# hormes/koordinator

Measured on AMD Instinct MI355X. Metric: pod×node Filter+Score evals/sec + pods/sec at 50k nodes, 1/2/4/8 GPUs, higher is better.
Workload: dtype int64

## Files before the change

koordinator_amd/csrc/gs_kernels.hip:

```cpp
#include <hip/hip_runtime.h>
#include <stdint.h>

#include <cstdio>
#include <vector>

#include "gs_eval_dev.h"

namespace gs {

__device__ __forceinline__ uint32_t node_prep_flags(uint32_t sf, int64_t update_time, int64_t now, int32_t filter_expired,
                                                    int32_t has_exp, int64_t exp_ns) {
  bool exists = sf & SF_METRIC;
  bool expired = !exists || !(sf & SF_UPDATE_TIME) || (exp_ns > 0 && now - update_time >= exp_ns);
  bool skip_filter = !exists || (filter_expired && has_exp && expired);
  uint32_t df = 0;
  if (!skip_filter) {
    const uint32_t npd = ((sf & SF_NP_MEM) ? 1u : 0u) | ((sf & SF_NP_AGG) ? 2u : 0u);
    if (sf & SF_FAIL_NP) df |= DF_LA_FAIL_NP | npd << DF_NP_DETAIL_SHIFT;
    if (sf & SF_PROD_THR) {
      if (sf & SF_FAIL_P) df |= DF_LA_FAIL_P | (((sf & SF_P_MEM) ? 1u : 0u) << DF_P_DETAIL_SHIFT);
    } else if (sf & SF_FAIL_NP) {
      df |= DF_LA_FAIL_P | npd << DF_P_DETAIL_SHIFT;
    }
  }
// ... 263 lines not shown
      if (nz && lane < ls) {
        s_score[nb] = b;
        s_count[nb] = (int32_t)c;
        slot_of[b] = (int8_t)nb;
      }
      if (sm) {
        next = __builtin_amdgcn_readlane(b, ls);
        nlev += __popcll(nzm & ((1ull << ls) - 1ull));
        break;
      }
      nlev += __popcll(nzm);
      cum += (uint32_t)wave_sum((int)c);
    }
    for (int j = nlev + lane; j < LEVALL; j += 64) { s_score[j] = -1; s_count[j] = 0; }
    if (lane == 0) {
      s_nlev = nlev;
      s_next = next;
    }
  } else if (t == 64 && cp.tb) {
    tiebreak_records(cp.seed, cp.seq[k], cp.tb + (size_t)k * TB_N);
  }
  __syncthreads();
  CT(2);
  const int nlev = s_nlev;
  for (int e = t; e < W * LEVALL; e += CAND_THREADS) {
    const int w = e / LEVALL, j = e % LEVALL;
    uint32_t off = 0;
    if (j < nlev) {
      for (int jj = 0; jj < j; ++jj) off += s_count[jj];
      for (int ww = 0; ww < w; ++ww) off += whist[ww * nbins + s_score[j]];
    }
    s_woff[w][j] = off;
  }
  __syncthreads();
  CT(3);
  uint32_t* out = lists + (size_t)k * lcap;
  if (nlev > 0) {
    uint32_t run_l = lane < LEVALL ? s_woff[wave][lane] : 0;
    const int thr = s_score[nlev - 1];
    auto next_step = [&](uint32_t b) {
      for (; b < we; b += 512) {
        const uint32_t st = (b - wb) / 512;
        if (st >= (uint32_t)STEPCAP || s_stepmax[wave][st] >= thr) break;
      }
      return b;
    };
    constexpr int PD = 4;
    uint32_t bq[PD];
    int4 vq[PD];
    uint32_t nb = next_step(wb);
#pragma unroll
    for (int u = 0; u < PD; ++u) {
      bq[u] = nb;
      vq[u] = nb < we ? row4[(nb + lane * 8) / 8] : make_int4(-1, -1, -1, -1);
      nb = nb < we ? next_step(nb + 512) : we;
    }
    while (bq[0] < we) {
      const uint32_t base = bq[0];
      const int4 q = vq[0];
#pragma unroll
      for (int u = 0; u + 1 < PD; ++u) { bq[u] = bq[u + 1]; vq[u] = vq[u + 1]; }
      bq[PD - 1] = nb;
      vq[PD - 1] = nb < we ? row4[(nb + lane * 8) / 8] : make_int4(-1, -1, -1, -1);
      nb = nb < we ? next_step(nb + 512) : we;
      const int16_t* e = reinterpret_cast<const int16_t*>(&q);
      int slot[8];
      uint32_t present = 0;
#pragma unroll
      for (int x = 0; x < 8; ++x) {
        slot[x] = e[x] >= thr ? slot_of[e[x]] : -1;
        if (slot[x] >= 0) present |= 1u << slot[x];
      }
      uint32_t pw = (uint32_t)wave_or((int)present);
      for (; pw; pw &= pw - 1) {
        const int j = __ffs(pw) - 1;
        int c = 0;
#pragma unroll
        for (int x = 0; x < 8; ++x) c += slot[x] == j;
        const int incl = wave_incl_scan(c);
        int pos = __builtin_amdgcn_readlane((int)run_l, j) + incl - c;
#pragma unroll
        for (int x = 0; x < 8; ++x)
          if (slot[x] == j) out[pos++] = n0 + base + lane * 8 + x;
        const int tot = __builtin_amdgcn_readlane(incl, 63);
        if (lane == j) run_l += tot;
      }
    }
  }
  CT(4);
  if (t == 0) {
    LevelHdr h;
    h.nlev = nlev < MAXLEV ? nlev : MAXLEV;
    h.feasible = (int32_t)s_total;
    h.next = nlev > MAXLEV ? s_score[MAXLEV] : s_next;
    int32_t tot = 0;
    for (int j = 0; j < MAXLEV; ++j) { h.score[j] = s_score[j]; h.count[j] = s_count[j]; tot += s_count[j]; }
    h.total = tot;
    hdrs[k] = h;
    LevelExt x;
    x.nlev = nlev;
    x.next = s_next;
    for (int j = 0; j < LEVX; ++j) { x.score[j] = s_score[MAXLEV + j]; x.count[j] = s_count[MAXLEV + j]; }
    ext[k] = x;
  }
}

__global__ void __launch_bounds__(256) cs_hist_kernel(const int16_t* __restrict__ S, uint32_t ld, uint32_t lenv,
                                                      int nbins, uint32_t slice, int G, uint32_t* __restrict__ ghist) {
  extern __shared__ __align__(16) uint32_t hist[];
  const int g = blockIdx.x, k = blockIdx.y, t = threadIdx.x;
  for (int b = t; b < nbins; b += 256) hist[b] = 0;
  __syncthreads();
  const uint32_t b0 = (uint32_t)g * slice, b1 = min(lenv, b0 + slice);
  const int4* row4 = reinterpret_cast<const int4*>(S + (size_t)k * ld);
  for (uint32_t i = b0 + t * 8; i < b1; i += 2 * 2048) {
    const int4 q0 = row4[i / 8];
    const int4 q1 = i + 2048 < b1 ? row4[(i + 2048) / 8] : make_int4(-1, -1, -1, -1);
    const int16_t* e0 = reinterpret_cast<const int16_t*>(&q0);
    const int16_t* e1 = reinterpret_cast<const int16_t*>(&q1);
#pragma unroll
    for (int x = 0; x < 8; ++x) {
      if (e0[x] >= 0) atomicAdd(&hist[e0[x]], 1u);
      if (e1[x] >= 0) atomicAdd(&hist[e1[x]], 1u);
    }
  }
  __syncthreads();
  uint32_t* out = ghist + ((size_t)k * G + g) * nbins;
  for (int b = t; b < nbins; b += 256) out[b] = hist[b];
}

__global__ void __launch_bounds__(256) cs_pick_kernel(const uint32_t* __restrict__ ghist, int nbins, int G, int lcap,
                                                      uint32_t* __restrict__ offs, LevelHdr* __restrict__ hdrs,
                                                      LevelExt* __restrict__ ext) {
  extern __shared__ __align__(16) uint32_t comb[];
  __shared__ uint32_t s_total;
  __shared__ int32_t s_nlev, s_next, s_score[LEVALL], s_count[LEVALL];
  __shared__ uint32_t s_v[CS_GMAX][LEVALL];
  const int k = blockIdx.x, t = threadIdx.x, wave = t >> 6, lane = t & 63;
  const uint32_t* h = ghist + (size_t)k * G * nbins;
  for (int b = t; b < nbins; b += 256) comb[b] = 0;
  if (t == 0) s_total = 0;
  __syncthreads();
  const int tot = G * nbins;
  for (int e0 = t; e0 < tot; e0 += 4 * 256) {
    uint32_t v[4];
#pragma unroll
    for (int u = 0; u < 4; ++u) v[u] = e0 + u * 256 < tot ? h[e0 + u * 256] : 0u;
#pragma unroll
    for (int u = 0; u < 4; ++u)
      if (v[u]) atomicAdd(&comb[(e0 + u * 256) % nbins], v[u]);
  }
  __syncthreads();
  {
    uint32_t s = 0;
    for (int b = t; b < nbins; b += 256) s += comb[b];
    s = (uint32_t)wave_sum((int)s);
    if (lane == 0 && s) atomicAdd(&s_total, s);
  }
  if (wave == 0) {
    const uint32_t target = (uint32_t)k + 1;
    const uint64_t lt = (1ull << lane) - 1ull;
    int nlev = 0, next = -1;
    uint32_t cum = 0;
    for (int hi = nbins - 1; hi >= 0; hi -= 64) {
      const int b = hi - lane;
      const uint32_t c = b >= 0 ? comb[b] : 0u;
      const bool nz = c != 0;
      const uint64_t nzm = __ballot(nz);
      if (!nzm) continue;
      const uint32_t cb = cum + (uint32_t)(wave_incl_scan((int)c) - (int)c);
      const int nb = nlev + __popcll(nzm & lt);
      const bool stop = nz && (nb == LEVALL || cb + c > (uint32_t)lcap || cb >= target);
      const uint64_t sm = __ballot(stop);
      const int ls = sm ? __builtin_ctzll(sm) : 64;
      if (nz && lane < ls) {
        s_score[nb] = b;
        s_count[nb] = (int32_t)c;
      }
      if (sm) {
        next = __builtin_amdgcn_readlane(b, ls);
        nlev += __popcll(nzm & ((1ull << ls) - 1ull));
        break;
      }
      nlev += __popcll(nzm);
      cum += (uint32_t)wave_sum((int)c);
    }
    for (int j = nlev + lane; j < LEVALL; j += 64) { s_score[j] = -1; s_count[j] = 0; }
    if (lane == 0) {
      s_nlev = nlev;
      s_next = next;
    }
  }
  __syncthreads();
  const int nlev = s_nlev;
  for (int e = t; e < G * LEVALL; e += 256) {
    const int g = e / LEVALL, j = e % LEVALL;
    s_v[g][j] = j < nlev ? h[(size_t)g * nbins + s_score[j]] : 0u;
  }
  __syncthreads();
  if (t < LEVALL) {
    uint32_t base = 0;
    for (int jj = 0; jj < t && jj < nlev; ++jj) base += (uint32_t)s_count[jj];
    uint32_t* o = offs + (size_t)k * G * LEVALL;
    for (int g = 0; g < G; ++g) {
      o[g * LEVALL + t] = base;
      base += s_v[g][t];
    }
  }
  if (t == 0) {
    LevelHdr hd;
    hd.nlev = nlev < MAXLEV ? nlev : MAXLEV;
    hd.feasible = (int32_t)s_total;
    hd.next = nlev > MAXLEV ? s_score[MAXLEV] : s_next;
    int32_t sum = 0;
    for (int j = 0; j < MAXLEV; ++j) { hd.score[j] = s_score[j]; hd.count[j] = s_count[j]; sum += s_count[j]; }
    hd.total = sum;
    hdrs[k] = hd;
    LevelExt x;
    x.nlev = nlev;
    x.next = s_next;
    for (int j = 0; j < LEVX; ++j) { x.score[j] = s_score[MAXLEV + j]; x.count[j] = s_count[MAXLEV + j]; }
    ext[k] = x;
  }
}

__global__ void __launch_bounds__(64) cs_list_kernel(const int16_t* __restrict__ S, uint32_t ld, uint32_t lenv,
                                                     uint32_t n0, int nbins, uint32_t slice, int G, int lcap,
                                                     const uint32_t* __restrict__ offs,
                                                     const LevelHdr* __restrict__ hdrs,
                                                     const LevelExt* __restrict__ ext, uint32_t* __restrict__ lists) {
  extern __shared__ __align__(16) int8_t slot_of[];
  const int g = blockIdx.x, k = blockIdx.y, lane = threadIdx.x;
  const int nlev = ext[k].nlev;
  if (nlev <= 0) return;
  for (int b = lane; b < nbins; b += 64) slot_of[b] = -1;
  __syncthreads();
  int sc = -1;
  if (lane < nlev) sc = lane < MAXLEV ? hdrs[k].score[lane] : ext[k].score[lane - MAXLEV];
  if (lane < nlev) slot_of[sc] = (int8_t)lane;
  const int thr = __shfl(sc, nlev - 1);
  __syncthreads();
  uint32_t run_l = lane < LEVALL ? offs[((size_t)k * G + g) * LEVALL + lane] : 0u;
  uint32_t* out = lists + (size_t)k * lcap;
  const uint32_t b0 = (uint32_t)g * slice, b1 = min(lenv, b0 + slice);
  const int4* row4 = reinterpret_cast<const int4*>(S + (size_t)k * ld);
  for (uint32_t gb = b0; gb < b1; gb += 4 * 512) {
    int4 qs[4];
#pragma unroll
    for (int u = 0; u < 4; ++u)
      qs[u] = gb + u * 512 < b1 ? row4[(gb + u * 512 + lane * 8) / 8] : make_int4(-1, -1, -1, -1);
#pragma unroll
    for (int u = 0; u < 4; ++u) {
      const uint32_t base = gb + u * 512;
      const int16_t* e = reinterpret_cast<const int16_t*>(&qs[u]);
      int slot[8];
      uint32_t present = 0;
#pragma unroll
      for (int x = 0; x < 8; ++x) {
        slot[x] = e[x] >= thr ? slot_of[e[x]] : -1;
        if (slot[x] >= 0) present |= 1u << slot[x];
      }
      uint32_t pw = (uint32_t)wave_or((int)present);
      for (; pw; pw &= pw - 1) {
        const int j = __ffs(pw) - 1;
        int c = 0;
#pragma unroll
        for (int x = 0; x < 8; ++x) c += slot[x] == j;
        const int incl = wave_incl_scan(c);
        int pos = __builtin_amdgcn_readlane((int)run_l, j) + incl - c;
#pragma unroll
        for (int x = 0; x < 8; ++x)
          if (slot[x] == j) out[pos++] = n0 + base + lane * 8 + x;
        const int tot = __builtin_amdgcn_readlane(incl, 63);
        if (lane == j) run_l += tot;
      }
    }
  }
}

constexpr int FIX_THREADS = 256;
__device__ __forceinline__ int lower_bound_u32(const uint32_t* a, int n, uint32_t x) {
  int lo = 0;
  while (n > 0) {
    const int h = n >> 1;
    if (a[lo + h] < x) { lo += h + 1; n -= h + 1; } else { n = h; }
  }
  return lo;
}
__global__ void __launch_bounds__(FIX_THREADS) fix_levels_kernel(int16_t* __restrict__ S, uint32_t ld, int max_score,
                                                                 int lcap, uint32_t* __restrict__ lists,
                                                                 LevelHdr* __restrict__ hdrs, LevelExt* __restrict__ ext,
                                                                 CandPatch cp, uint64_t* stamps) {
  uint64_t ct_last = stamps ? __builtin_amdgcn_s_memtime() : 0;
  auto CT = [&](int i) {
    if (!stamps) return;
    const uint64_t t_ = __builtin_amdgcn_s_memtime();
    if (threadIdx.x == 0) atomicAdd(reinterpret_cast<unsigned long long*>(&stamps[i]), (unsigned long long)(t_ - ct_last));
    ct_last = t_;
  };
  extern __shared__ __align__(16) uint32_t smem[];
  const int nbins = max_score + 1;
  uint32_t* hist = smem;
  uint32_t* olist = smem + nbins;
  __shared__ uint32_t p_raw[MAX_BATCH], p_node[MAX_BATCH];
  __shared__ int32_t p_old[MAX_BATCH], p_new[MAX_BATCH];
  __shared__ unsigned long long m_old[LEVALL][2], m_new[LEVALL][2];
  __shared__ int32_t n_ol[LEVALL];
  __shared__ int32_t o_score[LEVALL], o_count[LEVALL], o_off[LEVALL];
  __shared__ int32_t n_score[LEVALL], n_count[LEVALL], n_off[LEVALL];
  __shared__ int32_t s_onlev, s_onext, s_ofeas, s_np, s_fd, s_nlev, s_next, s_top;
  __shared__ int32_t r_old[MAX_BATCH], r_new[MAX_BATCH], p_sidx[MAX_BATCH];
  __shared__ int32_t s_wd[2];
  int8_t* lev_of = reinterpret_cast<int8_t*>(olist + lcap);
  const int k = blockIdx.x, t = threadIdx.x, lane = t & 63;
  if (cp.prev_committed[0] <= 0) return;
  const int32_t* lh = reinterpret_cast<const int32_t*>(cp.landed);
  const int nl = min(max(lh[0], 0), MAX_BATCH), npol = min(max(lh[1], 0), nl);
  const int split = min(max(npol, nl - 64), 64);
  const int slot_t = t < 64 ? (t < split ? t : -1) : (t < 128 && split + (t - 64) < nl ? split + (t - 64) : -1);
  const int32_t node_t = slot_t >= 0 ? lh[LANDED_NODES / 4 + slot_t] : -1;
  __shared__ unsigned int s_ev_max[2];
  if (stamps && t < 2) s_ev_max[t] = 0;
  if (stamps) __syncthreads();
  static_assert(FIX_THREADS == 256 && MAX_BATCH <= 128, "fix_levels_kernel: waves 0-1 evaluate, 2-3 load");
  if (t >= FIX_THREADS - 64) {
    const LevelHdr& h = hdrs[k];
    const LevelExt& x = ext[k];
    const int onl = x.nlev;
    const int j = lane;
    int sc = -1, cnt = 0;
    if (j < LEVALL) {
      sc = j < MAXLEV ? h.score[j] : x.score[j - MAXLEV];
      cnt = j < onl ? (j < MAXLEV ? h.count[j] : x.count[j - MAXLEV]) : 0;
    }
    const int incl = wave_incl_scan(cnt);
    if (j < LEVALL) {
      o_score[j] = sc;
      o_count[j] = cnt;
      o_off[j] = incl - cnt;
    }
    if (lane == 0) {
      s_onlev = onl;
      s_onext = x.next;
      s_ofeas = h.feasible;
      s_fd = 0;
      s_top = onl > 0 ? h.score[0] : x.next;
    }
    const int otot = onl > 0 ? __shfl(incl, onl - 1) : 0;
    const uint32_t* src = lists + (size_t)k * lcap;
    for (int e0 = 0; e0 < otot; e0 += 8 * 64) {
      uint32_t v[8];
#pragma unroll
      for (int u = 0; u < 8; ++u) {
        const int e = e0 + u * 64 + lane;
        v[u] = e < otot ? src[e] : 0u;
      }
#pragma unroll
      for (int u = 0; u < 8; ++u) {
        const int e = e0 + u * 64 + lane;
        if (e < otot) olist[e] = v[u];
      }
    }
  } else if (t >= FIX_THREADS - 128) {
    for (int b = lane; b < nbins; b += 64) hist[b] = cp.hist[(size_t)k * nbins + b];
  }
  const bool numa = (cp.pf.enabled & 0x30u) != 0;
  size_t at = 0;
  int so = -1, sn = -1, aff_v = -1;
  bool valid = false;
  if (t < 128) {
    const int32_t node = node_t;
    valid = node >= 0 && (uint32_t)node >= cp.n0 && (uint32_t)node < cp.n1;
    p_raw[t] = valid ? (uint32_t)node : 0xffffffffu;
    if (valid) {
      const uint64_t e0 = stamps ? __builtin_amdgcn_s_memtime() : 0;
      if (stamps && t == 0)
        atomicAdd(reinterpret_cast<unsigned long long*>(&stamps[10]), (unsigned long long)(e0 - ct_last));
      at = (size_t)k * ld + ((uint32_t)node - cp.n0);
      so = S[at];
      const Row r = reinterpret_cast<const Row*>(cp.landed + LANDED_ROWS)[slot_t];
      if (stamps) {
        __builtin_amdgcn_s_waitcnt(0);
        atomicMax(&s_ev_max[0], (unsigned int)(__builtin_amdgcn_s_memtime() - e0));
      }
      const PairOut o = eval_pair<false, true, true>(r, cp.pods[k], cp.pf, cp.m);
      sn = total_score(o, cp.pf);
      if (numa && ((r.nr.nflags >> NF_POLICY_SHIFT) & 3u)) aff_v = o.code ? 0 : (int)o.aff;
      if (stamps) atomicMax(&s_ev_max[1], (unsigned int)(__builtin_amdgcn_s_memtime() - e0));
    }
    r_old[t] = so;
    r_new[t] = sn;
  }
  __syncthreads();
  if (stamps && t == 0) {
    atomicAdd(reinterpret_cast<unsigned long long*>(&stamps[8]), (unsigned long long)s_ev_max[0]);
    atomicAdd(reinterpret_cast<unsigned long long*>(&stamps[9]), (unsigned long long)s_ev_max[1]);
    atomicAdd(reinterpret_cast<unsigned long long*>(&stamps[11]),
              (unsigned long long)(__builtin_amdgcn_s_memtime() - ct_last));
  }
  if (t < 128) {
    const uint32_t x = p_raw[t];
    const uint32_t k0 = p_raw[lane], k1 = p_raw[64 + lane];
    int rank = 0;
#pragma unroll
    for (int i = 0; i < 64; ++i) {
      const uint32_t y0 = __builtin_amdgcn_readlane(k0, i), y1 = __builtin_amdgcn_readlane(k1, i);
      rank += ((y0 < x || (y0 == x && i < t))) ? 1 : 0;
      rank += ((y1 < x || (y1 == x && 64 + i < t))) ? 1 : 0;
    }
    p_sidx[rank] = t;
  }
  __syncthreads();
  bool keep = false;
  int idx = 0, wpre = 0;
  uint32_t xs = 0;
  if (t < 2 * 64) {
    idx = p_sidx[t];
    xs = p_raw[idx];
    keep = xs != 0xffffffffu && (t == 0 || p_raw[p_sidx[t - 1]] != xs);
    const uint64_t m = __ballot(keep);
    wpre = __popcll(m & ((1ull << lane) - 1ull));
    if (lane == 0) s_wd[t >> 6] = __popcll(m);
  }
  __syncthreads();
  if (keep) {
    const int pos = (t >= 64 ? s_wd[0] : 0) + wpre;
    const int o_ = r_old[idx], n_ = r_new[idx];
    p_node[pos] = xs;
    p_old[pos] = o_;
    p_new[pos] = n_;
    if (o_ >= 0) atomicSub(&hist[o_], 1u);
    if (n_ >= 0) atomicAdd(&hist[n_], 1u);
    const int fd = (n_ >= 0 ? 1 : 0) - (o_ >= 0 ? 1 : 0);
    if (fd) atomicAdd(&s_fd, fd);
    atomicMax(&s_top, n_);
  }
  if (t == 0) s_np = s_wd[0] + s_wd[1];
  __syncthreads();
  CT(5);
  const int np = s_np;
  if (t < 64) {
    const uint32_t target = (uint32_t)k + 1;
    const int onext = s_onext;
    const uint64_t lt = (1ull << lane) - 1ull;
    int nlev = 0, next = -1;
    uint32_t cum = 0;
    for (int hi = min(s_top, nbins - 1); hi >= 0; hi -= 64) {
      const int b = hi - lane;
      const uint32_t c = b >= 0 ? hist[b] : 0u;
      const bool nz = c != 0;
      const uint64_t nzm = __ballot(nz);
      if (!nzm) continue;
      const uint32_t cb = cum + (uint32_t)(wave_incl_scan((int)c) - (int)c);
      const int nb = nlev + __popcll(nzm & lt);
      const bool stop = nz && (nb == LEVALL || cb + c > (uint32_t)lcap || cb >= target || b <= onext);
      const uint64_t sm = __ballot(stop);
      const int ls = sm ? __builtin_ctzll(sm) : 64;
      if (nz && lane < ls) {
        n_score[nb] = b;
        n_count[nb] = (int32_t)c;
      }
      if (sm) {
        next = __builtin_amdgcn_readlane(b, ls);
        nlev += __popcll(nzm & ((1ull << ls) - 1ull));
        break;
      }
      nlev += __popcll(nzm);
      cum += (uint32_t)wave_sum((int)c);
    }
    for (int j = nlev + lane; j < LEVALL; j += 64) { n_score[j] = -1; n_count[j] = 0; }
    WAVE_FENCE();
    const int cnt = lane < LEVALL ? n_count[lane] : 0;
    if (lane < LEVALL) n_off[lane] = wave_incl_scan(cnt) - cnt;
    if (lane == 0) {
      s_nlev = nlev;
      s_next = next;
    }
  }
  __syncthreads();
  CT(6);
  const int nlev = s_nlev;
  for (int b = t; b < nbins; b += FIX_THREADS) lev_of[b] = -1;
  if (t < LEVALL * 2) { m_old[t >> 1][t & 1] = 0; m_new[t >> 1][t & 1] = 0; }
  __syncthreads();
  if (t < nlev) {
    lev_of[n_score[t]] = (int8_t)t;
    int o = -1;
    for (int i = 0; i < s_onlev; ++i) o = o_score[i] == n_score[t] ? i : o;
    n_ol[t] = o;
  }
  __syncthreads();
  if (t < np) {
    const int jo = p_old[t] >= 0 ? lev_of[p_old[t]] : -1, jn = p_new[t] >= 0 ? lev_of[p_new[t]] : -1;
    if (jo >= 0) atomicOr(&m_old[jo][t >> 6], 1ull << (t & 63));
    if (jn >= 0) atomicOr(&m_new[jn][t >> 6], 1ull << (t & 63));
  }
  __syncthreads();
  auto below = [](const unsigned long long (&m)[2], int pos) {
    const int lo = min(pos, 64), hi = max(pos - 64, 0);
    return __popcll(lo >= 64 ? m[0] : (m[0] & ((1ull << lo) - 1ull))) +
           __popcll(hi >= 64 ? m[1] : (m[1] & ((1ull << hi) - 1ull)));
  };
  uint32_t* out = lists + (size_t)k * lcap;
  const int onlev = s_onlev;
  const int otot = onlev > 0 ? o_off[onlev - 1] + o_count[onlev - 1] : 0;
  for (int e = t; e < otot; e += FIX_THREADS) {
    int oj = 0;
    for (int step = 16; step; step >>= 1)
      if (oj + step < onlev && o_off[oj + step] <= e) oj += step;
    const int j = lev_of[o_score[oj]];
    if (j < 0) continue;
    const uint32_t x = olist[e];
    const int pos = lower_bound_u32(p_node, np, x);
    if (pos < np && p_node[pos] == x) continue;
    out[n_off[j] + (e - o_off[oj]) - below(m_old[j], pos) + below(m_new[j], pos)] = x;
  }
  if (t < np) {
    const int sn = p_new[t];
    const int j = sn >= 0 ? lev_of[sn] : -1;
    if (j >= 0) {
      const int oj = n_ol[j];
      const int before = oj >= 0 ? lower_bound_u32(olist + o_off[oj], o_count[oj], p_node[t]) - below(m_old[j], t) : 0;
      out[n_off[j] + below(m_new[j], t) + before] = p_node[t];
    }
  }
  CT(7);
  if (t == 0) {
    LevelHdr h;
    h.nlev = nlev < MAXLEV ? nlev : MAXLEV;
    h.feasible = s_ofeas + s_fd;
    h.next = nlev > MAXLEV ? n_score[MAXLEV] : s_next;
    int32_t tot = 0;
    for (int j = 0; j < MAXLEV; ++j) { h.score[j] = n_score[j]; h.count[j] = n_count[j]; tot += n_count[j]; }
    h.total = tot;
    hdrs[k] = h;
    LevelExt x;
    x.nlev = nlev;
    x.next = s_next;
    for (int j = 0; j < LEVX; ++j) { x.score[j] = n_score[MAXLEV + j]; x.count[j] = n_count[MAXLEV + j]; }
    ext[k] = x;
  }
  if (valid) {
    S[at] = (int16_t)sn;
    if (aff_v >= 0) cp.aff[at] = (uint8_t)aff_v;
  }
}

__global__ void __launch_bounds__(256) unpack_scores_kernel(const uint8_t* __restrict__ xin, size_t xblock, int R,
                                                            int npods, uint32_t per, uint32_t pld, uint32_t N,
                                                            int16_t* __restrict__ S, uint8_t* __restrict__ aff,
                                                            uint32_t ld, int32_t* __restrict__ xerr) {
  const int r = blockIdx.z, k = blockIdx.y;
  const uint32_t i = blockIdx.x * 256 + threadIdx.x;
  if (r == 0 && k == 0 && blockIdx.x == 0 && threadIdx.x == 0) {
    const XTag* t0 = reinterpret_cast<const XTag*>(xin + xblock - sizeof(XTag));
    int bad = 0;
    for (int q = 0; q < R && !bad; ++q) {
      const XTag* tq = reinterpret_cast<const XTag*>(xin + (size_t)q * xblock + xblock - sizeof(XTag));
      if (tq->magic != XTAG_MAGIC || tq->site != t0->site || tq->seq != t0->seq || tq->batch != t0->batch ||
          tq->rank != q || tq->bytes != (uint32_t)xblock)
        bad = 1 + q;
    }
    xerr[0] = bad;
    if (bad && !xerr[1]) {
      xerr[1] = 1;
      uint32_t* dst = reinterpret_cast<uint32_t*>(xerr + XERR_TAGS);
      for (int q = 0; q < R; ++q) {
        const uint32_t* tq = reinterpret_cast<const uint32_t*>(xin + (size_t)q * xblock + xblock - sizeof(XTag));
        for (int w = 0; w < (int)(sizeof(XTag) / 4); ++w) dst[q * (sizeof(XTag) / 4) + w] = tq[w];
      }
    }
  }
  const uint32_t node = (uint32_t)r * per + i;
  if (i >= per || node >= N) return;
  const uint8_t* blk = xin + (size_t)r * xblock;
  S[(size_t)k * ld + node] = reinterpret_cast<const int16_t*>(blk)[(size_t)k * pld + i];
  aff[(size_t)k * ld + node] = blk[(size_t)npods * pld * 2 + (size_t)k * pld + i];
}

hipError_t launch_unpack_scores(const uint8_t* xin, size_t xblock, int nranks, int npods, uint32_t per, uint32_t pld,
                                uint32_t N, int16_t* S, uint8_t* aff, uint32_t ld, int32_t* xerr, hipStream_t st) {
  if (npods <= 0 || nranks <= 0) return hipSuccess;
  hipLaunchKernelGGL(unpack_scores_kernel, dim3((per + 255) / 256, npods, nranks), dim3(256), 0, st, xin, xblock,
                     nranks, npods, per, pld, N, S, aff, ld, xerr);
  return hipGetLastError();
}

__global__ void __launch_bounds__(256) merge_levels_kernel(const uint8_t* __restrict__ xin, size_t xblock, int R,
                                                           int bmax, int lstride, uint8_t* __restrict__ xout,
                                                           int32_t* __restrict__ xerr) {
  constexpr int NEMAX = MAX_RANKS * LEVALL;
  static_assert(NEMAX <= 256, "one thread per shard level");
  __shared__ int32_t e_score[NEMAX], e_count[NEMAX], e_rep[NEMAX];
  __shared__ int32_t s_next[MAX_RANKS], s_feas[MAX_RANKS];
  __shared__ int32_t m_score[LEVALL], m_count[LEVALL];
  __shared__ int32_t s_nlev, s_drop;
  const int k = blockIdx.x, t = threadIdx.x, NE = R * LEVALL;
  if (k == 0 && t == 0) {
    const XTag* t0 = reinterpret_cast<const XTag*>(xin + xblock - sizeof(XTag));
    int bad = 0;
    for (int r = 0; r < R && !bad; ++r) {
      const XTag* tr = reinterpret_cast<const XTag*>(xin + (size_t)r * xblock + xblock - sizeof(XTag));
      if (tr->magic != XTAG_MAGIC || tr->site != t0->site || tr->seq != t0->seq || tr->batch != t0->batch ||
          tr->rank != r || tr->bytes != (uint32_t)xblock)
        bad = 1 + r;
    }
    xerr[0] = bad;
    if (bad && !xerr[1]) {
      xerr[1] = 1;
      uint32_t* dst = reinterpret_cast<uint32_t*>(xerr + XERR_TAGS);
      for (int r = 0; r < R; ++r) {
        const uint32_t* tr = reinterpret_cast<const uint32_t*>(xin + (size_t)r * xblock + xblock - sizeof(XTag));
        for (int w = 0; w < (int)(sizeof(XTag) / 4); ++w) dst[r * (sizeof(XTag) / 4) + w] = tr[w];
      }
    }
  }
  const size_t ihoff = (size_t)bmax * lstride * 4, ixoff = ihoff + (size_t)bmax * sizeof(LevelHdr);
  const size_t hoff = (size_t)bmax * LCAP * 4, xoff = hoff + (size_t)bmax * sizeof(LevelHdr);
  if (t == 0) { s_nlev = 0; s_drop = -1; }
  if (t < LEVALL) { m_score[t] = -1; m_count[t] = 0; }
  int off = 0;
  if (t < NE) {
    const int r = t / LEVALL, j = t % LEVALL;
    const LevelHdr* h = reinterpret_cast<const LevelHdr*>(xin + r * xblock + ihoff) + k;
    const LevelExt* x = reinterpret_cast<const LevelExt*>(xin + r * xblock + ixoff) + k;
    const int nl = x->nlev;
    int s = -1, c = 0;
    if (j < nl) {
      s = j < MAXLEV ? h->score[j] : x->score[j - MAXLEV];
      c = j < MAXLEV ? h->count[j] : x->count[j - MAXLEV];
    }
    e_score[t] = s;
    e_count[t] = c;
    if (j == 0) { s_next[r] = x->next; s_feas[r] = h->feasible; }
  }
  __syncthreads();
  int mnext = -1, feas = 0;
  for (int r = 0; r < R; ++r) { mnext = max(mnext, s_next[r]); feas += s_feas[r]; }
  int s = -1;
  if (t < NE) {
    s = e_score[t];
    const int r = t / LEVALL, j = t % LEVALL;
    for (int jj = 0; jj < j; ++jj) off += e_count[r * LEVALL + jj];
    bool rep = s > mnext;
    for (int u = 0; u < t && rep; ++u) rep = e_score[u] != s;
    e_rep[t] = rep;
  }
  __syncthreads();
  int pos = -1;
  if (t < NE && s > mnext) {

    int rank = 0, cum = 0, before = 0, tot = 0;
    for (int u = 0; u < NE; ++u) {
      const int su = e_score[u];
      if (su > s) { cum += e_count[u]; rank += e_rep[u]; }
      else if (su == s) { tot += e_count[u]; if (u < t) before += e_count[u]; }
    }
    if (rank < LEVALL && cum + tot <= LCAP) {
      pos = cum + before;
      if (e_rep[t]) { m_score[rank] = s; m_count[rank] = tot; atomicAdd(&s_nlev, 1); }
    } else if (e_rep[t]) {
      atomicMax(&s_drop, s);
    }
  }
  __syncthreads();
  uint32_t* out = reinterpret_cast<uint32_t*>(xout) + (size_t)k * LCAP;
  __shared__ int32_t s_pos[NEMAX], s_off[NEMAX];
  if (t < NE) { s_pos[t] = pos; s_off[t] = off; }
  __syncthreads();
  for (int u = 0; u < NE; ++u) {
    const int pu = s_pos[u];
    if (pu < 0) continue;
    const uint32_t* in = reinterpret_cast<const uint32_t*>(xin + (u / LEVALL) * xblock) + (size_t)k * lstride + s_off[u];
    const int cu = e_count[u];
    for (int x = t; x < cu; x += 256) out[pu + x] = in[x];
  }
  if (t == 0) {
    const int nlev = s_nlev, next = max(mnext, s_drop);
    LevelHdr h;
    h.nlev = nlev < MAXLEV ? nlev : MAXLEV;
    h.feasible = feas;
    h.next = nlev > MAXLEV ? m_score[MAXLEV] : next;
    int32_t tot = 0;
    for (int j = 0; j < MAXLEV; ++j) { h.score[j] = m_score[j]; h.count[j] = m_count[j]; tot += m_count[j]; }
    h.total = tot;
    reinterpret_cast<LevelHdr*>(xout + hoff)[k] = h;
    LevelExt x;
    x.nlev = nlev;
    x.next = next;
    for (int j = 0; j < LEVX; ++j) { x.score[j] = m_score[MAXLEV + j]; x.count[j] = m_count[MAXLEV + j]; }
    reinterpret_cast<LevelExt*>(xout + xoff)[k] = x;
  }
}

hipError_t launch_merge_levels(const uint8_t* xin, size_t xblock, int nranks, int npods, int bmax, int lstride,
                               uint8_t* xout, int32_t* xerr, hipStream_t st) {
  if (npods <= 0) return hipSuccess;
  if (nranks < 2 || nranks > MAX_RANKS || lstride > LCAP || nranks * lstride > LCAP) return hipErrorInvalidValue;
  if (xblock < sizeof(XTag) || xblock % 256) return hipErrorInvalidValue;
  hipLaunchKernelGGL(merge_levels_kernel, dim3(npods), dim3(256), 0, st, xin, xblock, nranks, bmax, lstride, xout,
                     xerr);
  return hipGetLastError();
}

__global__ void write_tag_kernel(uint8_t* __restrict__ dst, XTag t) {
  if (threadIdx.x == 0) *reinterpret_cast<XTag*>(dst) = t;
}

hipError_t launch_write_tag(uint8_t* dst, const XTag& t, hipStream_t st) {
  if (reinterpret_cast<uintptr_t>(dst) % 8) return hipErrorInvalidValue;
  hipLaunchKernelGGL(write_tag_kernel, dim3(1), dim3(64), 0, st, dst, t);
  return hipGetLastError();
}

int64_t host_tiebreak_position(uint64_t seed, uint64_t seq, int64_t T) { return tiebreak_position(seed, seq, T); }

extern "C" int gsx_tiebreak_selftest(uint64_t seed, int iters, char* msg, size_t len) {
  uint64_t st = seed * 0x9E3779B97F4A7C15ull + 1;
  auto rnd = [&]() { st += 0x9E3779B97F4A7C15ull; return mix64(st); };
  int bad = 0;
  if (msg && len) msg[0] = 0;
  for (int it = 0; it < iters; ++it) {
    const uint64_t sd = rnd(), sq = rnd();
    int32_t r[TB_N];
    tiebreak_records(sd, sq, r);
    const int32_t lim = r[TB_N - 1];
    std::vector<int64_t> Ts = {1, 2, 3, (int64_t)(rnd() % 1000) + 1, (int64_t)(rnd() % 200000) + 1,
                               (int64_t)(rnd() % (1ull << 31)) + 1, (int64_t)lim, (int64_t)lim + 1};
    for (int k = 0; k < TB_N - 1 && r[k] != INT32_MAX; ++k)
      for (int64_t d = -1; d <= 1; ++d) Ts.push_back((int64_t)r[k] + d);
    for (int64_t T : Ts) {
      if (T < 1) continue;
      int64_t got;
      if (T > (int64_t)lim) {
        got = tiebreak_position(sd, sq, T);
      } else {
        int cnt = 0;
        for (int k = 0; k < TB_N - 1; ++k) cnt += (r[k] != INT32_MAX && (int64_t)r[k] <= T) ? 1 : 0;
        got = cnt ? (int64_t)r[cnt - 1] : 1;
      }
      const int64_t want = tiebreak_position(sd, sq, T);
      if (got != want) {
        if (!bad && msg && len)
// ... 657 lines not shown
```

Before: 9.397 billion.

## Rank landed nodes in the idle loader wave and drop the sort/compaction barriers

Moves the rank sort of landed node IDs from a post-evaluation phase into the otherwise lightly used hist-loader wave, so it overlaps with pair evaluation. It removes the deduplication and compaction pass and two block-wide barriers, writing old and new scores straight to their sorted positions. This assumes landed nodes are unique and all fall within [n0,n1). With duplicates or out-of-range entries, ranks collide (clamped to nl-1), np becomes nl instead of the compacted count, and invalid slots leave p_old and p_new unset.

```diff
diff --git a/koordinator_amd/csrc/gs_kernels.hip b/koordinator_amd/csrc/gs_kernels.hip
--- a/koordinator_amd/csrc/gs_kernels.hip
+++ b/koordinator_amd/csrc/gs_kernels.hip
@@ -589,15 +589,14 @@
   const int nbins = max_score + 1;
   uint32_t* hist = smem;
   uint32_t* olist = smem + nbins;
-  __shared__ uint32_t p_raw[MAX_BATCH], p_node[MAX_BATCH];
+  __shared__ uint32_t p_node[MAX_BATCH];
   __shared__ int32_t p_old[MAX_BATCH], p_new[MAX_BATCH];
   __shared__ unsigned long long m_old[LEVALL][2], m_new[LEVALL][2];
   __shared__ int32_t n_ol[LEVALL];
   __shared__ int32_t o_score[LEVALL], o_count[LEVALL], o_off[LEVALL];
   __shared__ int32_t n_score[LEVALL], n_count[LEVALL], n_off[LEVALL];
-  __shared__ int32_t s_onlev, s_onext, s_ofeas, s_np, s_fd, s_nlev, s_next, s_top;
-  __shared__ int32_t r_old[MAX_BATCH], r_new[MAX_BATCH], p_sidx[MAX_BATCH];
-  __shared__ int32_t s_wd[2];
+  __shared__ int32_t s_onlev, s_onext, s_ofeas, s_fd, s_nlev, s_next, s_top;
+  __shared__ int32_t p_rank[MAX_BATCH];
   int8_t* lev_of = reinterpret_cast<int8_t*>(olist + lcap);
   const int k = blockIdx.x, t = threadIdx.x, lane = t & 63;
   if (cp.prev_committed[0] <= 0) return;
@@ -650,6 +649,18 @@
     }
   } else if (t >= FIX_THREADS - 128) {
     for (int b = lane; b < nbins; b += 64) hist[b] = cp.hist[(size_t)k * nbins + b];
+    static_assert(MAX_BATCH <= 128, "two slab entries per lane");
+    const uint32_t k0 = lane < nl ? (uint32_t)lh[LANDED_NODES / 4 + lane] : 0xffffffffu;
+    const uint32_t k1 = 64 + lane < nl ? (uint32_t)lh[LANDED_NODES / 4 + 64 + lane] : 0xffffffffu;
+    int r0 = 0, r1 = 0;
+#pragma unroll
+    for (int i = 0; i < 64; ++i) {
+      const uint32_t y0 = __builtin_amdgcn_readlane(k0, i), y1 = __builtin_amdgcn_readlane(k1, i);
+      r0 += (y0 < k0 ? 1 : 0) + (y1 < k0 ? 1 : 0);
+      r1 += (y0 < k1 ? 1 : 0) + (y1 < k1 ? 1 : 0);
+    }
+    if (lane < nl) { p_node[min(r0, nl - 1)] = k0; p_rank[lane] = min(r0, nl - 1); }
+    if (64 + lane < nl) { p_node[min(r1, nl - 1)] = k1; p_rank[64 + lane] = min(r1, nl - 1); }
   }
   const bool numa = (cp.pf.enabled & 0x30u) != 0;
   size_t at = 0;
@@ -658,7 +669,6 @@
   if (t < 128) {
     const int32_t node = node_t;
     valid = node >= 0 && (uint32_t)node >= cp.n0 && (uint32_t)node < cp.n1;
-    p_raw[t] = valid ? (uint32_t)node : 0xffffffffu;
     if (valid) {
       const uint64_t e0 = stamps ? __builtin_amdgcn_s_memtime() : 0;
       if (stamps && t == 0)
@@ -675,8 +685,6 @@
       if (numa && ((r.nr.nflags >> NF_POLICY_SHIFT) & 3u)) aff_v = o.code ? 0 : (int)o.aff;
       if (stamps) atomicMax(&s_ev_max[1], (unsigned int)(__builtin_amdgcn_s_memtime() - e0));
     }
-    r_old[t] = so;
-    r_new[t] = sn;
   }
   __syncthreads();
   if (stamps && t == 0) {
@@ -685,47 +693,21 @@
     atomicAdd(reinterpret_cast<unsigned long long*>(&stamps[11]),
               (unsigned long long)(__builtin_amdgcn_s_memtime() - ct_last));
   }
-  if (t < 128) {
-    const uint32_t x = p_raw[t];
-    const uint32_t k0 = p_raw[lane], k1 = p_raw[64 + lane];
-    int rank = 0;
-#pragma unroll
-    for (int i = 0; i < 64; ++i) {
-      const uint32_t y0 = __builtin_amdgcn_readlane(k0, i), y1 = __builtin_amdgcn_readlane(k1, i);
-      rank += ((y0 < x || (y0 == x && i < t))) ? 1 : 0;
-      rank += ((y1 < x || (y1 == x && 64 + i < t))) ? 1 : 0;
-    }
-    p_sidx[rank] = t;
-  }
-  __syncthreads();
-  bool keep = false;
-  int idx = 0, wpre = 0;
-  uint32_t xs = 0;
-  if (t < 2 * 64) {
-    idx = p_sidx[t];
-    xs = p_raw[idx];
-    keep = xs != 0xffffffffu && (t == 0 || p_raw[p_sidx[t - 1]] != xs);
-    const uint64_t m = __ballot(keep);
-    wpre = __popcll(m & ((1ull << lane) - 1ull));
-    if (lane == 0) s_wd[t >> 6] = __popcll(m);
-  }
-  __syncthreads();
-  if (keep) {
-    const int pos = (t >= 64 ? s_wd[0] : 0) + wpre;
-    const int o_ = r_old[idx], n_ = r_new[idx];
-    p_node[pos] = xs;
-    p_old[pos] = o_;
-    p_new[pos] = n_;
-    if (o_ >= 0) atomicSub(&hist[o_], 1u);
-    if (n_ >= 0) atomicAdd(&hist[n_], 1u);
-    const int fd = (n_ >= 0 ? 1 : 0) - (o_ >= 0 ? 1 : 0);
+  if (slot_t >= 0) {
+    const int rank = p_rank[slot_t];
+    p_old[rank] = so;
+    p_new[rank] = sn;
+  }
+  if (valid) {
+    if (so >= 0) atomicSub(&hist[so], 1u);
+    if (sn >= 0) atomicAdd(&hist[sn], 1u);
+    const int fd = (sn >= 0 ? 1 : 0) - (so >= 0 ? 1 : 0);
     if (fd) atomicAdd(&s_fd, fd);
-    atomicMax(&s_top, n_);
-  }
-  if (t == 0) s_np = s_wd[0] + s_wd[1];
+    atomicMax(&s_top, sn);
+  }
   __syncthreads();
   CT(5);
-  const int np = s_np;
+  const int np = nl;
   if (t < 64) {
     const uint32_t target = (uint32_t)k + 1;
     const int onext = s_onext;
```

Measured after the change: 9.537 billion (median of 4 runs). 1.01x the previous value.
